# indrajeetadityaroy9/vit-bias-aware-structural-distillation

Measured on AMD Instinct MI355X. Metric: images/sec BASD train step, DeiT-T student / ViT-B teacher bs=256, higher is better.
Workload: dtype bf16; 1 GPU; BASELINE configs[1]: DeiT-Tiny/16 student, ViT-Base/16 teacher (random init), 224x224, E=4 extraction points, loss linalg fp32/fp64; global_batch=256, per_gpu_batch=256, parallelism=dp1, grad_checkpointing=False

## Files before the change

### vit-bias-aware-structural-distillation_amd/csrc/token_gram.hip

```cpp
#include "basd_frag.h"

namespace basd {

constexpr int TM = 64;
constexpr int KC = 32;
constexpr int XS = KC + 2;
constexpr int MAXCT = 8;

__device__ __forceinline__ int nct_tiles(int d_out) { const int n = d_out >> 4; return n * (n + 1) / 2; }

template <typename T>
__device__ __forceinline__ float ld_as_f32(const T* p);
template <> __device__ __forceinline__ float ld_as_f32<float>(const float* p) { return *p; }
template <> __device__ __forceinline__ float ld_as_f32<unsigned short>(const unsigned short* p) {
  return bf16_bits_to_f32(*p);
}

template <typename T, int MAXGT>
__global__ __launch_bounds__(512) void token_gram_kernel(const T* __restrict__ x, int64_t rows, int d_in,
                                                         int rows_per_batch, int64_t batch_stride,
                                                         const float* __restrict__ proj, int d_out,
                                                         double* __restrict__ gram,
                                                         double* __restrict__ colsum) {
  extern __shared__ __align__(16) float sm[];
  const int ldz = d_out + 16;
  float* Xs = sm;
  float* Ps = Xs + TM * XS;
  float* Z = Ps + d_out * XS;
  __shared__ unsigned char s_it[136], s_jt[136];
  const int tid = threadIdx.x, lane = tid & 63, wave = tid >> 6;
  const int nct = d_out >> 4;
  const int rt = wave & 3;
  const int ct0 = (wave >> 2) * ((nct + 1) >> 1);
  const int ct1 = (wave >> 2) ? nct : ((nct + 1) >> 1);
  const int ngt = nct * (nct + 1) / 2;

  for (int g = threadIdx.x; g < nct_tiles(d_out); g += 512) {
    int it = 0;
    while ((it + 1) * (it + 2) / 2 <= g) ++it;
    s_it[g] = (unsigned char)it;
    s_jt[g] = (unsigned char)(g - it * (it + 1) / 2);
  }
  __syncthreads();
  f64x4 gacc[MAXGT];
#pragma unroll
  for (int i = 0; i < MAXGT; ++i) gacc[i] = (f64x4){0.0, 0.0, 0.0, 0.0};
  double csum = 0.0;

  const int64_t ntiles = (rows + TM - 1) / TM;
  for (int64_t tile = blockIdx.x; tile < ntiles; tile += gridDim.x) {
    const int64_t r0 = tile * TM;
    f32x4 zacc[MAXCT];
#pragma unroll
    for (int i = 0; i < MAXCT; ++i) zacc[i] = (f32x4){0.f, 0.f, 0.f, 0.f};
    for (int k0 = 0; k0 < d_in; k0 += KC) {
      __syncthreads();
      for (int i = tid; i < TM * KC; i += 512) {
        const int r = i / KC, k = i - r * KC;
        const int64_t gr = r0 + r;
        const int64_t gb = gr / rows_per_batch;
        Xs[r * XS + k] = (gr < rows) ? ld_as_f32<T>(x + gb * batch_stride + (gr - gb * rows_per_batch) * d_in + k0 + k) : 0.f;
      }
      for (int i = tid; i < d_out * KC; i += 512) {
        const int r = i / KC, k = i - r * KC;
        Ps[r * XS + k] = proj[(size_t)r * d_in + k0 + k];
      }
      __syncthreads();
#pragma unroll 2
      for (int kk = 0; kk < KC / 4; ++kk) {
        const float a = Xs[(rt * 16 + (lane & 15)) * XS + kk * 4 + (lane >> 4)];
#pragma unroll
        for (int c = 0; c < MAXCT; ++c) {
          const int ct = ct0 + c;
          if (ct < ct1) {
            const float b = Ps[(ct * 16 + (lane & 15)) * XS + kk * 4 + (lane >> 4)];
            zacc[c] = __builtin_amdgcn_mfma_f32_16x16x4f32(a, b, zacc[c], 0, 0, 0);
          }
        }
      }
    }
#pragma unroll
    for (int c = 0; c < MAXCT; ++c) {
      const int ct = ct0 + c;
      if (ct < ct1) {
#pragma unroll
        for (int reg = 0; reg < 4; ++reg)
          Z[(rt * 16 + (lane >> 4) * 4 + reg) * ldz + ct * 16 + (lane & 15)] = zacc[c][reg];
      }
    }
    __syncthreads();
    if (tid < d_out) {
      double s = 0.0;
      for (int r = 0; r < TM; ++r) s += (double)Z[r * ldz + tid];
      csum += s;
    }
#pragma unroll
    for (int gi = 0; gi < MAXGT; ++gi) {
      const int g = wave + gi * 8;
      if (g < ngt) {
        const int it = s_it[g], jt = s_jt[g];
#pragma unroll 2
        for (int kk = 0; kk < TM / 4; ++kk) {
          const float* zr = Z + (kk * 4 + (lane >> 4)) * ldz + (lane & 15);
          const double a = (double)zr[it * 16];
          const double b = (double)zr[jt * 16];
          gacc[gi] = __builtin_amdgcn_mfma_f64_16x16x4f64(a, b, gacc[gi], 0, 0, 0);
        }
      }
    }
  }
#pragma unroll
  for (int gi = 0; gi < MAXGT; ++gi) {
    const int g = wave + gi * 8;
    if (g < ngt) {
      const int it = s_it[g], jt = s_jt[g];
#pragma unroll
      for (int reg = 0; reg < 4; ++reg) {
        const int i = it * 16 + (lane >> 4) + 4 * reg;
        const int j = jt * 16 + (lane & 15);
        const double v = gacc[gi][reg];
        atomicAdd(&gram[(size_t)i * d_out + j], v);
      }
    }
  }
  if (tid < d_out) atomicAdd(&colsum[tid], csum);
}

}

extern "C" int basd_token_gram(const void* x, int x_dtype, int64_t rows, int d_in, int rows_per_batch,
                               int64_t batch_stride, const float* proj, int d_out, double* gram, double* colsum,
                               void* stream) {
  using namespace basd;
  if (rows <= 0) return BASD_OK;
  if (rows_per_batch < 1) return fail(BASD_ERR_SHAPE, "token_gram: rows_per_batch < 1");
  if (d_out < 16 || d_out > 256 || d_out % 16 || d_in < KC || d_in % KC)
    return fail(BASD_ERR_SHAPE, "token_gram: need d_out %% 16 == 0, 16 <= d_out <= 256, d_in %% %d == 0 (got %d, %d)",
                KC, d_out, d_in);
  const size_t lds = (size_t)(TM * XS + d_out * XS + TM * (d_out + 16)) * 4;
  const int64_t ntiles = (rows + TM - 1) / TM;
  const int grid = (int)(ntiles < 256 ? ntiles : 256);
  hipStream_t st = (hipStream_t)stream;
#define BASD_TG_LAUNCH(T, G)                                                                        \
  do {                                                                                              \
    allow_full_lds((const void*)token_gram_kernel<T, G>);                                           \
    hipLaunchKernelGGL((token_gram_kernel<T, G>), dim3(grid), dim3(512), lds, st, (const T*)x, rows, d_in, \
                       rows_per_batch, batch_stride, proj, d_out, gram, colsum);                                                  \
  } while (0)
  if (x_dtype == BASD_DTYPE_F32) {
    if (d_out <= 192) BASD_TG_LAUNCH(float, 10); else BASD_TG_LAUNCH(float, 17);
  } else if (x_dtype == BASD_DTYPE_BF16) {
    if (d_out <= 192) BASD_TG_LAUNCH(unsigned short, 10); else BASD_TG_LAUNCH(unsigned short, 17);
  } else {
    return fail(BASD_ERR_DTYPE, "token_gram: dtype %d", x_dtype);
  }
#undef BASD_TG_LAUNCH
  return check_launch("token_gram");
}

namespace basd {

constexpr int TM2 = 128;
constexpr int KC2 = 32;
constexpr int PROW = 80;

template <int NCT>
__global__ __launch_bounds__(256) void token_gram_bf16x3_kernel(const unsigned short* __restrict__ x, int64_t rows,
                                                                int d_in, int rows_per_batch, int64_t batch_stride,
                                                                const unsigned short* __restrict__ psplit,
                                                                double* __restrict__ gram,
                                                                double* __restrict__ colsum) {
  constexpr int D_OUT = NCT * 16;
  constexpr int LDZ = D_OUT + 16;
  constexpr int NGT = NCT * (NCT + 1) / 2;
  constexpr int GT_PER_WAVE = (NGT + 3) / 4;
  extern __shared__ __align__(16) unsigned char smem[];
  unsigned char* Pl = smem;
  float* Z = reinterpret_cast<float*>(smem);
  __shared__ unsigned char s_it[NGT], s_jt[NGT];
  const int tid = threadIdx.x, lane = tid & 63, wave = tid >> 6;
  for (int g = tid; g < NGT; g += 256) {
    int it = 0;
    while ((it + 1) * (it + 2) / 2 <= g) ++it;
    s_it[g] = (unsigned char)it;
    s_jt[g] = (unsigned char)(g - it * (it + 1) / 2);
  }
  f64x4 gacc[GT_PER_WAVE];
#pragma unroll
  for (int i = 0; i < GT_PER_WAVE; ++i) gacc[i] = (f64x4){0.0, 0.0, 0.0, 0.0};
  double csum = 0.0;
  const size_t split_stride = (size_t)D_OUT * d_in;

  const int64_t ntiles = (rows + TM2 - 1) / TM2;
  for (int64_t tile = blockIdx.x; tile < ntiles; tile += gridDim.x) {
    const int64_t r0 = tile * TM2 + wave * 32;
    f32x4 zacc[2][NCT];
#pragma unroll
    for (int g = 0; g < 2; ++g)
#pragma unroll
      for (int c = 0; c < NCT; ++c) zacc[g][c] = (f32x4){0.f, 0.f, 0.f, 0.f};
    const int64_t ra = r0 + (lane & 15), rb = ra + 16;
    const int64_t ba = ra / rows_per_batch, bb = rb / rows_per_batch;
    const unsigned short* xa = x + ba * batch_stride + (ra - ba * rows_per_batch) * d_in + 8 * (lane >> 4);
    const unsigned short* xb = x + bb * batch_stride + (rb - bb * rows_per_batch) * d_in + 8 * (lane >> 4);
    constexpr int PVEC = (3 * D_OUT * 4 + 255) / 256;
    uint4 pre[PVEC];
    bf16x8 a0n, a1n;
    auto fetch = [&](int k0) {
#pragma unroll
      for (int v = 0; v < PVEC; ++v) {
        const int e = tid + 256 * v;
        const int q = e & 3, rc = e >> 2;
        const int sp = rc / D_OUT, col = rc - sp * D_OUT;
        pre[v] = (rc < 3 * D_OUT)
                     ? *reinterpret_cast<const uint4*>(psplit + sp * split_stride + (size_t)col * d_in + k0 + 8 * q)
                     : make_uint4(0, 0, 0, 0);
      }
      a0n = (bf16x8){0, 0, 0, 0, 0, 0, 0, 0};
      a1n = a0n;
      if (ra < rows) a0n = *reinterpret_cast<const bf16x8*>(xa + k0);
      if (rb < rows) a1n = *reinterpret_cast<const bf16x8*>(xb + k0);
    };
    auto stash = [&](unsigned char* buf) {
#pragma unroll
      for (int v = 0; v < PVEC; ++v) {
        const int e = tid + 256 * v;
        const int q = e & 3, rc = e >> 2;
        if (rc < 3 * D_OUT) *reinterpret_cast<uint4*>(buf + (size_t)rc * PROW + 16 * q) = pre[v];
      }
    };
    constexpr size_t PBUF = (size_t)3 * D_OUT * PROW;
    __syncthreads();
    fetch(0);
    stash(Pl);
    bf16x8 a0 = a0n, a1 = a1n;
    __syncthreads();
    int cur = 0;
    for (int k0 = 0; k0 < d_in; k0 += KC2) {
      const bool more = k0 + KC2 < d_in;
      if (more) fetch(k0 + KC2);
      const unsigned char* Pc = Pl + cur * PBUF;
#pragma unroll
      for (int s = 0; s < 3; ++s) {
#pragma unroll
        for (int c = 0; c < NCT; ++c) {
          const bf16x8 b = *reinterpret_cast<const bf16x8*>(
              Pc + (size_t)(s * D_OUT + c * 16 + (lane & 15)) * PROW + 16 * (lane >> 4));
          zacc[0][c] = __builtin_amdgcn_mfma_f32_16x16x32_bf16(a0, b, zacc[0][c], 0, 0, 0);
          zacc[1][c] = __builtin_amdgcn_mfma_f32_16x16x32_bf16(a1, b, zacc[1][c], 0, 0, 0);
        }
      }
      if (more) {
        stash(Pl + (cur ^ 1) * PBUF);
        a0 = a0n; a1 = a1n;
      }
      cur ^= 1;
      __syncthreads();
    }
    __syncthreads();
#pragma unroll
    for (int g = 0; g < 2; ++g)
#pragma unroll
      for (int c = 0; c < NCT; ++c)
#pragma unroll
        for (int reg = 0; reg < 4; ++reg)
          Z[(wave * 32 + g * 16 + (lane >> 4) * 4 + reg) * LDZ + c * 16 + (lane & 15)] = zacc[g][c][reg];
    __syncthreads();
    const int64_t rows_left = rows - tile * TM2;
    const int nvalid = rows_left < TM2 ? (int)rows_left : TM2;
    float* mu = Z + (size_t)TM2 * LDZ;
    double* wv = reinterpret_cast<double*>(mu + D_OUT);
    if (tid < D_OUT) {
      double sacc = 0.0;
      for (int r = 0; r < TM2; ++r) sacc += (double)Z[r * LDZ + tid];
      const float m_ = (float)(sacc / (double)nvalid);
      mu[tid] = m_;
      wv[tid] = sacc - 0.5 * (double)nvalid * (double)m_;
      csum += sacc;
    }
    __syncthreads();
    for (int e = tid; e < nvalid * D_OUT; e += 256) {
      const int r = e / D_OUT, c = e - r * D_OUT;
      Z[r * LDZ + c] -= mu[c];
    }
    __syncthreads();
#pragma unroll
    for (int gi = 0; gi < GT_PER_WAVE; ++gi) {
      const int g = wave + gi * 4;
      if (g < NGT) {
        const int it = s_it[g], jt = s_jt[g];
        f32x4 t = {0.f, 0.f, 0.f, 0.f};
#pragma unroll 8
        for (int kk = 0; kk < TM2 / 4; ++kk) {
          const float* zr = Z + (kk * 4 + (lane >> 4)) * LDZ + (lane & 15);
          t = __builtin_amdgcn_mfma_f32_16x16x4f32(zr[it * 16], zr[jt * 16], t, 0, 0, 0);
        }
        {
          typedef unsigned int tg_u32x2 __attribute__((ext_vector_type(2)));
          tg_u32x2 a02 = __builtin_amdgcn_permlane32_swap(__float_as_uint(t[0]), __float_as_uint(t[2]), false, false);
          tg_u32x2 a13 = __builtin_amdgcn_permlane32_swap(__float_as_uint(t[1]), __float_as_uint(t[3]), false, false);
          tg_u32x2 b01 = __builtin_amdgcn_permlane16_swap(a02[0], a13[0], false, false);
          tg_u32x2 b23 = __builtin_amdgcn_permlane16_swap(a02[1], a13[1], false, false);
          gacc[gi][0] += (double)__uint_as_float(b01[0]);
          gacc[gi][1] += (double)__uint_as_float(b01[1]);
          gacc[gi][2] += (double)__uint_as_float(b23[0]);
          gacc[gi][3] += (double)__uint_as_float(b23[1]);
        }
        const int ks = lane >> 4;
        const double mi = (double)mu[it * 16 + (lane & 15)], mj = (double)mu[jt * 16 + (lane & 15)];
        const double wi = wv[it * 16 + (lane & 15)], wj = wv[jt * 16 + (lane & 15)];
        const double ai = ks == 0 ? mi : ks == 1 ? wi : 0.0;
        const double bj = ks == 0 ? wj : ks == 1 ? mj : 0.0;
        gacc[gi] = __builtin_amdgcn_mfma_f64_16x16x4f64(ai, bj, gacc[gi], 0, 0, 0);
      }
    }
  }
#pragma unroll
  for (int gi = 0; gi < GT_PER_WAVE; ++gi) {
    const int g = wave + gi * 4;
    if (g < NGT) {
      const int it = s_it[g], jt = s_jt[g];
#pragma unroll
      for (int reg = 0; reg < 4; ++reg) {
        const int i = it * 16 + (lane >> 4) + 4 * reg;
        const int j = jt * 16 + (lane & 15);
        const double v = gacc[gi][reg];
        atomicAdd(&gram[(size_t)i * D_OUT + j], v);
      }
    }
  }
  if (tid < D_OUT) atomicAdd(&colsum[tid], csum);
}

template <int NCT>
__global__ __launch_bounds__(256) void token_gram_bf16x3_t256_kernel(const unsigned short* __restrict__ x, int64_t rows,
                                                                int d_in, int rows_per_batch, int64_t batch_stride,
                                                                const unsigned short* __restrict__ psplit,
                                                                double* __restrict__ gram,
                                                                double* __restrict__ colsum) {
  constexpr int D_OUT = NCT * 16;
  constexpr int LDZ = D_OUT + 16;
  constexpr int NGT = NCT * (NCT + 1) / 2;
  constexpr int GT_PER_WAVE = (NGT + 3) / 4;
  extern __shared__ __align__(16) unsigned char smem[];
  unsigned char* Pl = smem;
  float* Z = reinterpret_cast<float*>(smem);
  __shared__ unsigned char s_it[NGT], s_jt[NGT];
  const int tid = threadIdx.x, lane = tid & 63, wave = tid >> 6;
  for (int g = tid; g < NGT; g += 256) {
    int it = 0;
    while ((it + 1) * (it + 2) / 2 <= g) ++it;
    s_it[g] = (unsigned char)it;
    s_jt[g] = (unsigned char)(g - it * (it + 1) / 2);
  }
  double csum = 0.0;
  const size_t split_stride = (size_t)D_OUT * d_in;
  __syncthreads();

  const int64_t ntiles = (rows + 2 * TM2 - 1) / (2 * TM2);
  for (int64_t tile = blockIdx.x; tile < ntiles; tile += gridDim.x) {
    f32x4 zacc[4][NCT];
#pragma unroll
    for (int g = 0; g < 4; ++g)
#pragma unroll
      for (int c = 0; c < NCT; ++c) zacc[g][c] = (f32x4){0.f, 0.f, 0.f, 0.f};
    const unsigned short* xr[4];
    bool rok[4];
#pragma unroll
    for (int g = 0; g < 4; ++g) {
      const int64_t r = tile * (2 * TM2) + (g >> 1) * TM2 + wave * 32 + (g & 1) * 16 + (lane & 15);
      rok[g] = r < rows;
      const int64_t rr = rok[g] ? r : 0;
      const int64_t bq = rr / rows_per_batch;
      xr[g] = x + bq * batch_stride + (rr - bq * rows_per_batch) * d_in + 8 * (lane >> 4);
    }
    constexpr int PVEC = (3 * D_OUT * 4 + 255) / 256;
    uint4 pre[PVEC];
    bf16x8 an[4];
    auto fetch = [&](int k0) {
#pragma unroll
      for (int v = 0; v < PVEC; ++v) {
        const int e = tid + 256 * v;
        const int q = e & 3, rc = e >> 2;
        const int sp = rc / D_OUT, col = rc - sp * D_OUT;
        pre[v] = (rc < 3 * D_OUT)
                     ? *reinterpret_cast<const uint4*>(psplit + sp * split_stride + (size_t)col * d_in + k0 + 8 * q)
                     : make_uint4(0, 0, 0, 0);
      }
#pragma unroll
      for (int g = 0; g < 4; ++g) {
        an[g] = (bf16x8){0, 0, 0, 0, 0, 0, 0, 0};
        if (rok[g]) an[g] = *reinterpret_cast<const bf16x8*>(xr[g] + k0);
      }
    };
    auto stash = [&](unsigned char* buf) {
#pragma unroll
      for (int v = 0; v < PVEC; ++v) {
        const int e = tid + 256 * v;
        const int q = e & 3, rc = e >> 2;
        if (rc < 3 * D_OUT) *reinterpret_cast<uint4*>(buf + (size_t)rc * PROW + 16 * q) = pre[v];
      }
    };
    constexpr size_t PBUF = (size_t)3 * D_OUT * PROW;
    __syncthreads();
    fetch(0);
    stash(Pl);
    bf16x8 ac[4];
#pragma unroll
    for (int g = 0; g < 4; ++g) ac[g] = an[g];
    __syncthreads();
    int cur = 0;
    for (int k0 = 0; k0 < d_in; k0 += KC2) {
      const bool more = k0 + KC2 < d_in;
      if (more) fetch(k0 + KC2);
      const unsigned char* Pc = Pl + cur * PBUF;
#pragma unroll
      for (int s_ = 0; s_ < 3; ++s_) {
#pragma unroll
        for (int c = 0; c < NCT; ++c) {
          const bf16x8 b = *reinterpret_cast<const bf16x8*>(
              Pc + (size_t)(s_ * D_OUT + c * 16 + (lane & 15)) * PROW + 16 * (lane >> 4));
#pragma unroll
          for (int g = 0; g < 4; ++g) zacc[g][c] = __builtin_amdgcn_mfma_f32_16x16x32_bf16(ac[g], b, zacc[g][c], 0, 0, 0);
        }
      }
      if (more) {
        stash(Pl + (cur ^ 1) * PBUF);
#pragma unroll
        for (int g = 0; g < 4; ++g) ac[g] = an[g];
      }
      cur ^= 1;
      __syncthreads();
    }
    f64x4 gacc[GT_PER_WAVE];
#pragma unroll
    for (int i = 0; i < GT_PER_WAVE; ++i) gacc[i] = (f64x4){0.0, 0.0, 0.0, 0.0};
#pragma unroll
    for (int pass = 0; pass < 2; ++pass) {
    const int64_t rows_left = rows - (tile * (2 * TM2) + pass * TM2);
    if (rows_left <= 0) break;
    __syncthreads();
#pragma unroll
    for (int g = 0; g < 2; ++g)
#pragma unroll
      for (int c = 0; c < NCT; ++c)
#pragma unroll
        for (int reg = 0; reg < 4; ++reg)
          Z[(wave * 32 + g * 16 + (lane >> 4) * 4 + reg) * LDZ + c * 16 + (lane & 15)] = zacc[2 * pass + g][c][reg];
    __syncthreads();
    const int nvalid = rows_left < TM2 ? (int)rows_left : TM2;
    float* mu = Z + (size_t)TM2 * LDZ;
    double* wv = reinterpret_cast<double*>(mu + D_OUT);
    if (tid < D_OUT) {
      double sacc = 0.0;
      for (int r = 0; r < TM2; ++r) sacc += (double)Z[r * LDZ + tid];
      const float m_ = (float)(sacc / (double)nvalid);
      mu[tid] = m_;
      wv[tid] = sacc - 0.5 * (double)nvalid * (double)m_;
      csum += sacc;
    }
    __syncthreads();
    for (int e = tid; e < nvalid * D_OUT; e += 256) {
      const int r = e / D_OUT, c = e - r * D_OUT;
      Z[r * LDZ + c] -= mu[c];
    }
    __syncthreads();
#pragma unroll
    for (int gi = 0; gi < GT_PER_WAVE; ++gi) {
      const int g = wave + gi * 4;
      if (g < NGT) {
        const int it = s_it[g], jt = s_jt[g];
        f32x4 t = {0.f, 0.f, 0.f, 0.f};
#pragma unroll 8
        for (int kk = 0; kk < TM2 / 4; ++kk) {
          const float* zr = Z + (kk * 4 + (lane >> 4)) * LDZ + (lane & 15);
          t = __builtin_amdgcn_mfma_f32_16x16x4f32(zr[it * 16], zr[jt * 16], t, 0, 0, 0);
        }
        {
          typedef unsigned int tg_u32x2 __attribute__((ext_vector_type(2)));
          tg_u32x2 a02 = __builtin_amdgcn_permlane32_swap(__float_as_uint(t[0]), __float_as_uint(t[2]), false, false);
          tg_u32x2 a13 = __builtin_amdgcn_permlane32_swap(__float_as_uint(t[1]), __float_as_uint(t[3]), false, false);
          tg_u32x2 b01 = __builtin_amdgcn_permlane16_swap(a02[0], a13[0], false, false);
          tg_u32x2 b23 = __builtin_amdgcn_permlane16_swap(a02[1], a13[1], false, false);
          gacc[gi][0] += (double)__uint_as_float(b01[0]);
          gacc[gi][1] += (double)__uint_as_float(b01[1]);
          gacc[gi][2] += (double)__uint_as_float(b23[0]);
          gacc[gi][3] += (double)__uint_as_float(b23[1]);
        }
        const int ks = lane >> 4;
        const double mi = (double)mu[it * 16 + (lane & 15)], mj = (double)mu[jt * 16 + (lane & 15)];
        const double wi = wv[it * 16 + (lane & 15)], wj = wv[jt * 16 + (lane & 15)];
        const double ai = ks == 0 ? mi : ks == 1 ? wi : 0.0;
        const double bj = ks == 0 ? wj : ks == 1 ? mj : 0.0;
        gacc[gi] = __builtin_amdgcn_mfma_f64_16x16x4f64(ai, bj, gacc[gi], 0, 0, 0);
      }
    }
    }
#pragma unroll
    for (int gi = 0; gi < GT_PER_WAVE; ++gi) {
      const int g = wave + gi * 4;
      if (g < NGT) {
        const int it = s_it[g], jt = s_jt[g];
#pragma unroll
        for (int reg = 0; reg < 4; ++reg) {
          const int i = it * 16 + (lane >> 4) + 4 * reg;
          const int j = jt * 16 + (lane & 15);
          atomicAdd(&gram[(size_t)i * D_OUT + j], gacc[gi][reg]);
        }
      }
    }
  }
  if (tid < D_OUT) atomicAdd(&colsum[tid], csum);
}

template <int NCT>
static void launch_tg_bf16x3(const void* x, int64_t rows, int d_in, int rows_per_batch, int64_t batch_stride,
                             const void* psplit, double* gram, double* colsum, hipStream_t st) {
  constexpr int D_OUT = NCT * 16;
  const size_t p_bytes = (size_t)2 * 3 * D_OUT * PROW;
  const size_t z_bytes = (size_t)TM2 * (D_OUT + 16) * 4 + (size_t)D_OUT * 12;
  const size_t lds = p_bytes > z_bytes ? p_bytes : z_bytes;
  const int64_t ntiles = (rows + TM2 - 1) / TM2;
  if (ntiles > 256) {
    const int64_t nt2 = (rows + 2 * TM2 - 1) / (2 * TM2);
    const int grid2 = (int)(nt2 < 256 ? nt2 : 256);
    allow_full_lds((const void*)token_gram_bf16x3_t256_kernel<NCT>);
    hipLaunchKernelGGL((token_gram_bf16x3_t256_kernel<NCT>), dim3(grid2), dim3(256), lds, st, (const unsigned short*)x, rows,
                       d_in, rows_per_batch, batch_stride, (const unsigned short*)psplit, gram, colsum);
    return;
  }
  const int grid = (int)(ntiles < 256 ? ntiles : 256);
  allow_full_lds((const void*)token_gram_bf16x3_kernel<NCT>);
  hipLaunchKernelGGL((token_gram_bf16x3_kernel<NCT>), dim3(grid), dim3(256), lds, st, (const unsigned short*)x, rows,
                     d_in, rows_per_batch, batch_stride, (const unsigned short*)psplit, gram, colsum);
}

}

extern "C" int basd_token_gram_bf16x3(const void* x, int64_t rows, int d_in, int rows_per_batch, int64_t batch_stride,
                                      const void* proj_split, int d_out, double* gram, double* colsum,
                                      void* stream) {
  using namespace basd;
  if (rows <= 0) return BASD_OK;
  if (rows_per_batch < 1) return fail(BASD_ERR_SHAPE, "token_gram_bf16x3: rows_per_batch < 1");
  if (d_in % KC2 || d_in < KC2) return fail(BASD_ERR_SHAPE, "token_gram_bf16x3: d_in %% 32 != 0 (%d)", d_in);
  if ((((uintptr_t)x) & 15) || batch_stride % 8)
    return fail(BASD_ERR_SHAPE, "token_gram_bf16x3: need a 16-byte aligned x and batch_stride %% 8 == 0 (got %lld)",
                (long long)batch_stride);
  hipStream_t st = (hipStream_t)stream;
  switch (d_out) {
    case 32: launch_tg_bf16x3<2>(x, rows, d_in, rows_per_batch, batch_stride, proj_split, gram, colsum, st); break;
    case 64: launch_tg_bf16x3<4>(x, rows, d_in, rows_per_batch, batch_stride, proj_split, gram, colsum, st); break;
    case 128: launch_tg_bf16x3<8>(x, rows, d_in, rows_per_batch, batch_stride, proj_split, gram, colsum, st); break;
    case 192: launch_tg_bf16x3<12>(x, rows, d_in, rows_per_batch, batch_stride, proj_split, gram, colsum, st); break;
    default: return fail(BASD_ERR_SHAPE, "token_gram_bf16x3: d_out %d not in {32, 64, 128, 192}", d_out);
  }
  return check_launch("token_gram_bf16x3");
}

namespace basd {

constexpr int GW_TR = 64;
constexpr int GW_BC = 128;
constexpr int GW_LD = GW_BC + 16;

__global__ __launch_bounds__(256) __attribute__((amdgpu_waves_per_eu(2, 2))) void gram_wide_f32_kernel(const float* __restrict__ z, int64_t rows, int d, int nbc,
                                                            int rsplit, double* __restrict__ gram,
                                                            double* __restrict__ colsum) {
  extern __shared__ __align__(16) float gw_lds[];
  float* Pi = gw_lds;
  float* Pj = Pi + GW_TR * GW_LD;
  float* mu = Pj + GW_TR * GW_LD;
  double* wv = reinterpret_cast<double*>(mu + 256);
  const int tid = threadIdx.x, lane = tid & 63, wave = tid >> 6;
  const int blk = blockIdx.x / rsplit, rs = blockIdx.x - blk * rsplit;
  int bi = 0;
  while ((bi + 1) * (bi + 2) / 2 <= blk) ++bi;
  const int bj = blk - bi * (bi + 1) / 2;
  const bool diag = bi == bj;
  const int ci0 = bi * GW_BC, cj0 = bj * GW_BC;
  const int64_t ntile = (rows + GW_TR - 1) / GW_TR;
  const int64_t t_lo = ntile * rs / rsplit, t_hi = ntile * (rs + 1) / rsplit;
  f64x4 acc[2][8];
#pragma unroll
  for (int a = 0; a < 2; ++a)
#pragma unroll
    for (int b = 0; b < 8; ++b) acc[a][b] = (f64x4){0.0, 0.0, 0.0, 0.0};
  double csum = 0.0;
  const int sr = tid >> 5, sq = tid & 31;
  float4 pre_i[8], pre_j[8];
  auto fetch = [&](int64_t tile) {
    const int64_t r0 = tile * GW_TR;
#pragma unroll
    for (int p = 0; p < 8; ++p) {
      const int64_t r = r0 + sr + 8 * p;
      const bool ok = r < rows;
      const float* src = z + (ok ? r : 0) * (int64_t)d;
      const bool oki = ok && ci0 + 4 * sq < d, okj = ok && cj0 + 4 * sq < d;
      pre_i[p] = oki ? *reinterpret_cast<const float4*>(src + ci0 + 4 * sq) : make_float4(0.f, 0.f, 0.f, 0.f);
      if (!diag) pre_j[p] = okj ? *reinterpret_cast<const float4*>(src + cj0 + 4 * sq) : make_float4(0.f, 0.f, 0.f, 0.f);
    }
  };
  for (int64_t tile = t_lo; tile < t_hi; ++tile) {
    fetch(tile);
    __syncthreads();
#pragma unroll
    for (int p = 0; p < 8; ++p) {
      *reinterpret_cast<float4*>(Pi + (sr + 8 * p) * GW_LD + 4 * sq) = pre_i[p];
      if (!diag) *reinterpret_cast<float4*>(Pj + (sr + 8 * p) * GW_LD + 4 * sq) = pre_j[p];
    }
    __syncthreads();
    const int64_t left = rows - tile * GW_TR;
    const int nvalid = left < GW_TR ? (int)left : GW_TR;
    {
      const float* col = (tid < 128 ? Pi : (diag ? Pi : Pj)) + (tid & 127);
      double s = 0.0;
#pragma unroll 8
      for (int r = 0; r < GW_TR; ++r) s += (double)col[r * GW_LD];
      const float m_ = (float)(s / (double)nvalid);
      mu[tid] = m_;
      wv[tid] = s - 0.5 * (double)nvalid * (double)m_;
      if (diag && tid < 128) csum += s;
    }
    __syncthreads();
    const float* Pjj = diag ? Pi : Pj;
    const int li = lane & 15, kq = lane >> 4;
    const bool partial = nvalid < GW_TR;
#pragma unroll
    for (int a = 0; a < 2; ++a) {
      const int it = 2 * wave + a;
      const float mi = mu[it * 16 + li];
      float af[GW_TR / 4];
#pragma unroll
      for (int kk = 0; kk < GW_TR / 4; ++kk) {
        const int r = kk * 4 + kq;
        const float v = Pi[r * GW_LD + it * 16 + li] - mi;
        af[kk] = (partial && r >= nvalid) ? 0.f : v;
      }
      double mi_r[4], wi_r[4];
#pragma unroll
      for (int reg = 0; reg < 4; ++reg) { mi_r[reg] = (double)mu[it * 16 + 4 * kq + reg]; wi_r[reg] = wv[it * 16 + 4 * kq + reg]; }
#pragma unroll
      for (int jp = 0; jp < 4; ++jp) {
        const int j0 = 2 * jp, j1 = 2 * jp + 1;
        if (diag && j0 > it) continue;
        const bool use1 = !(diag && j1 > it);
        const float mj0 = mu[128 + j0 * 16 + li], mj1 = mu[128 + j1 * 16 + li];
        f32x4 t0 = {0.f, 0.f, 0.f, 0.f}, t1 = {0.f, 0.f, 0.f, 0.f};
#pragma unroll
        for (int kk = 0; kk < GW_TR / 4; ++kk) {
          const int r = kk * 4 + kq;
          float b0 = Pjj[r * GW_LD + j0 * 16 + li] - mj0, b1 = Pjj[r * GW_LD + j1 * 16 + li] - mj1;
          if (partial && r >= nvalid) { b0 = 0.f; b1 = 0.f; }
          t0 = __builtin_amdgcn_mfma_f32_16x16x4f32(af[kk], b0, t0, 0, 0, 0);
          t1 = __builtin_amdgcn_mfma_f32_16x16x4f32(af[kk], b1, t1, 0, 0, 0);
        }
        const double wj0 = wv[128 + j0 * 16 + li], wj1 = wv[128 + j1 * 16 + li];
#pragma unroll
        for (int reg = 0; reg < 4; ++reg) {
          acc[a][j0][reg] += (double)t0[reg] + mi_r[reg] * wj0 + wi_r[reg] * (double)mj0;
          if (use1) acc[a][j1][reg] += (double)t1[reg] + mi_r[reg] * wj1 + wi_r[reg] * (double)mj1;
        }
      }
    }
  }
  const int li = lane & 15, kq = lane >> 4;
#pragma unroll
  for (int a = 0; a < 2; ++a) {
    const int it = 2 * wave + a;
#pragma unroll
    for (int jt = 0; jt < 8; ++jt) {
      if (diag && jt > it) continue;
#pragma unroll
      for (int reg = 0; reg < 4; ++reg) {
        const int gi = ci0 + it * 16 + 4 * kq + reg, gj = cj0 + jt * 16 + li;
        if (gi < d && gj < d) atomicAdd(&gram[(size_t)gi * d + gj], acc[a][jt][reg]);
      }
    }
  }
  if (diag && tid < 128 && ci0 + tid < d) atomicAdd(&colsum[ci0 + tid], csum);
}

}

extern "C" int basd_gram_f32_centred(const float* z, int64_t rows, int d, double* gram, double* colsum, void* stream) {
  using namespace basd;
  if (rows <= 0) return BASD_OK;
  if (d < 16 || d % 16 || d > 4096 || (((uintptr_t)z) & 15))
    return fail(BASD_ERR_SHAPE, "gram_f32_centred: need d %% 16 == 0, 16 <= d <= 4096, 16-byte aligned z (d=%d)", d);
  const int nbc = (d + GW_BC - 1) / GW_BC;
  const int nblk = nbc * (nbc + 1) / 2;
  const int64_t ntile = (rows + GW_TR - 1) / GW_TR;
  int rsplit = 512 / nblk;
  if ((int64_t)rsplit > ntile / 8) rsplit = (int)(ntile / 8);
  if (rsplit < 1) rsplit = 1;
  const size_t lds = (size_t)2 * GW_TR * GW_LD * 4 + 256 * 4 + 256 * 8;
  allow_full_lds((const void*)gram_wide_f32_kernel);
  hipLaunchKernelGGL(gram_wide_f32_kernel, dim3(nblk * rsplit), dim3(256), lds, (hipStream_t)stream, z, rows, d, nbc,
                     rsplit, gram, colsum);
  return check_launch("gram_f32_centred");
}
```

Baseline: 8247 images/sec.

## Stream projection tiles into LDS with direct global-to-LDS loads in a three-stage ring

Replaces the register-staged double buffer for the projection split in the large-row token Gram kernel with a three-stage LDS ring. The ring is filled by global_load_lds_dwordx4 DMA using an XOR-swizzled layout, and x fragments are loaded through inline asm with counted vmcnt waits. The intent is to stop projection data passing through VGPRs and ds_write, and to overlap the next chunk's loads with the MFMAs using one barrier per chunk. In exchange it relies on fragile inline asm, m0 manipulation and manual scheduling barriers, needs more LDS, and adds a cap on d_in.

```diff
diff --git a/vit-bias-aware-structural-distillation_amd/csrc/token_gram.hip b/vit-bias-aware-structural-distillation_amd/csrc/token_gram.hip
--- a/vit-bias-aware-structural-distillation_amd/csrc/token_gram.hip
+++ b/vit-bias-aware-structural-distillation_amd/csrc/token_gram.hip
@@ -1,3 +1,4 @@
+#include <type_traits>
 #include "basd_frag.h"
 
 namespace basd {
@@ -332,6 +333,15 @@
   if (tid < D_OUT) atomicAdd(&colsum[tid], csum);
 }
 
+constexpr int TG_NS = 3;
+
+__device__ __forceinline__ int tg_swz(int byte) { return byte ^ (((byte >> 9) & 1) << 5); }
+
+template <int N>
+__device__ __forceinline__ void tg_wait_pieces(u32x4 (&x)[4]) {
+  asm volatile("s_waitcnt vmcnt(%4)" : "+v"(x[0]), "+v"(x[1]), "+v"(x[2]), "+v"(x[3]) : "n"(N) : "memory");
+}
+
 template <int NCT>
 __global__ __launch_bounds__(256) void token_gram_bf16x3_t256_kernel(const unsigned short* __restrict__ x, int64_t rows,
                                                                 int d_in, int rows_per_batch, int64_t batch_stride,
@@ -342,8 +352,12 @@
   constexpr int LDZ = D_OUT + 16;
   constexpr int NGT = NCT * (NCT + 1) / 2;
   constexpr int GT_PER_WAVE = (NGT + 3) / 4;
+  constexpr int NP = 3 * NCT;
+  constexpr int NPW = (NP + 3) / 4;
+  constexpr int STAGE = NP * 1024;
+  static_assert(TG_NS == 3, "the issue order and the counted wait of the chunk loop are written for three stages");
+  static_assert(2 * NPW + 4 < 64, "vmcnt is a 6-bit counter");
   extern __shared__ __align__(16) unsigned char smem[];
-  unsigned char* Pl = smem;
   float* Z = reinterpret_cast<float*>(smem);
   __shared__ unsigned char s_it[NGT], s_jt[NGT];
   const int tid = threadIdx.x, lane = tid & 63, wave = tid >> 6;
@@ -354,7 +368,18 @@
     s_jt[g] = (unsigned char)(g - it * (it + 1) / 2);
   }
   double csum = 0.0;
-  const size_t split_stride = (size_t)D_OUT * d_in;
+  const int wave_u = __builtin_amdgcn_readfirstlane(wave);
+  const unsigned int lds_base = (unsigned int)(size_t)smem;
+  const unsigned char* pbytes = reinterpret_cast<const unsigned char*>(psplit);
+  const int q_dma = tg_swz(lane * 16);
+  int piece[NPW];
+  unsigned int poff[NPW];
+#pragma unroll
+  for (int j = 0; j < NPW; ++j) {
+    piece[j] = (wave_u + 4 * j) % NP;
+    poff[j] = (unsigned int)(((piece[j] * 16 + (q_dma >> 6)) * (size_t)d_in + ((q_dma >> 4) & 3) * 8) * 2);
+  }
+  const int frag_off = tg_swz((lane & 15) * 64 + (lane >> 4) * 16);
   __syncthreads();
 
   const int64_t ntiles = (rows + 2 * TM2 - 1) / (2 * TM2);
@@ -374,64 +399,73 @@
       const int64_t bq = rr / rows_per_batch;
       xr[g] = x + bq * batch_stride + (rr - bq * rows_per_batch) * d_in + 8 * (lane >> 4);
     }
-    constexpr int PVEC = (3 * D_OUT * 4 + 255) / 256;
-    uint4 pre[PVEC];
-    bf16x8 an[4];
-    auto fetch = [&](int k0) {
-#pragma unroll
-      for (int v = 0; v < PVEC; ++v) {
-        const int e = tid + 256 * v;
-        const int q = e & 3, rc = e >> 2;
-        const int sp = rc / D_OUT, col = rc - sp * D_OUT;
-        pre[v] = (rc < 3 * D_OUT)
-                     ? *reinterpret_cast<const uint4*>(psplit + sp * split_stride + (size_t)col * d_in + k0 + 8 * q)
-                     : make_uint4(0, 0, 0, 0);
-      }
+    u32x4 xn[4];
+    auto load_x = [&](int k0) {
+#pragma unroll
+      for (int g = 0; g < 4; ++g)
+        asm volatile("global_load_dwordx4 %0, %1, off" : "=v"(xn[g]) : "v"(xr[g] + k0) : "memory");
+    };
+    auto issue_piece = [&](int j, int stage, const unsigned char* base_u) {
+      const unsigned int dst = lds_base + stage * STAGE + piece[j] * 1024;
+      unsigned int keep;
+      asm volatile("s_mov_b32 %0, m0\n\ts_nop 3\n\ts_mov_b32 m0, %3\n\ts_nop 0\n\tglobal_load_lds_dwordx4 %1, %2\n\ts_mov_b32 m0, %0"
+                   : "=&s"(keep) : "v"(poff[j]), "s"(base_u), "s"(dst) : "memory");
+    };
+    const int nchunks = d_in / KC2;
+    asm volatile("s_waitcnt vmcnt(0)" ::: "memory");
+    __syncthreads();
+    {
+      const int c1 = nchunks > 1 ? 1 : 0;
+#pragma unroll
+      for (int j = 0; j < NPW; ++j) issue_piece(j, 0, pbytes);
+      load_x(0);
+#pragma unroll
+      for (int j = 0; j < NPW; ++j) issue_piece(j, 1, pbytes + (size_t)c1 * (KC2 * 2));
+    }
+    int st = 0;
+#pragma nounroll
+    for (int c = 0; c < nchunks; ++c) {
+      tg_wait_pieces<NPW>(xn);
+      __builtin_amdgcn_s_barrier();
+      __builtin_amdgcn_sched_barrier(0);
+      bf16x8 ac[4];
 #pragma unroll
       for (int g = 0; g < 4; ++g) {
-        an[g] = (bf16x8){0, 0, 0, 0, 0, 0, 0, 0};
-        if (rok[g]) an[g] = *reinterpret_cast<const bf16x8*>(xr[g] + k0);
-      }
-    };
-    auto stash = [&](unsigned char* buf) {
-#pragma unroll
-      for (int v = 0; v < PVEC; ++v) {
-        const int e = tid + 256 * v;
-        const int q = e & 3, rc = e >> 2;
-        if (rc < 3 * D_OUT) *reinterpret_cast<uint4*>(buf + (size_t)rc * PROW + 16 * q) = pre[v];
-      }
-    };
-    constexpr size_t PBUF = (size_t)3 * D_OUT * PROW;
-    __syncthreads();
-    fetch(0);
-    stash(Pl);
-    bf16x8 ac[4];
-#pragma unroll
-    for (int g = 0; g < 4; ++g) ac[g] = an[g];
-    __syncthreads();
-    int cur = 0;
-    for (int k0 = 0; k0 < d_in; k0 += KC2) {
-      const bool more = k0 + KC2 < d_in;
-      if (more) fetch(k0 + KC2);
-      const unsigned char* Pc = Pl + cur * PBUF;
-#pragma unroll
-      for (int s_ = 0; s_ < 3; ++s_) {
-#pragma unroll
-        for (int c = 0; c < NCT; ++c) {
-          const bf16x8 b = *reinterpret_cast<const bf16x8*>(
-              Pc + (size_t)(s_ * D_OUT + c * 16 + (lane & 15)) * PROW + 16 * (lane >> 4));
-#pragma unroll
-          for (int g = 0; g < 4; ++g) zacc[g][c] = __builtin_amdgcn_mfma_f32_16x16x32_bf16(ac[g], b, zacc[g][c], 0, 0, 0);
-        }
-      }
-      if (more) {
-        stash(Pl + (cur ^ 1) * PBUF);
-#pragma unroll
-        for (int g = 0; g < 4; ++g) ac[g] = an[g];
-      }
-      cur ^= 1;
-      __syncthreads();
-    }
+        const u32x4 v = rok[g] ? xn[g] : (u32x4){0u, 0u, 0u, 0u};
+        ac[g] = __builtin_bit_cast(bf16x8, v);
+      }
+      const int cx = c + 1 < nchunks ? c + 1 : nchunks - 1, cp = c + 2 < nchunks ? c + 2 : nchunks - 1;
+      load_x(cx * KC2);
+      const int stn = st == 0 ? TG_NS - 1 : st - 1;
+      const unsigned char* base_n = pbytes + (size_t)cp * (KC2 * 2);
+      const unsigned char* Pc = smem + st * STAGE + frag_off;
+      bf16x8 bq[2][4];
+      auto read_block = [&](bf16x8 (&q)[4], int b) {
+#pragma unroll
+        for (int i = 0; i < 4; ++i)
+          if (4 * b + i < NP) q[i] = *reinterpret_cast<const bf16x8*>(Pc + (4 * b + i) * 1024);
+      };
+      read_block(bq[0], 0);
+#pragma unroll
+      for (int b = 0; b < NPW; ++b) {
+        __builtin_amdgcn_sched_barrier(0);
+        issue_piece(b, stn, base_n);
+        if (b + 1 < NPW) read_block(bq[(b + 1) & 1], b + 1);
+        __builtin_amdgcn_sched_barrier(0);
+#pragma unroll
+        for (int i = 0; i < 4; ++i) {
+          const int t = 4 * b + i;
+          if (t < NP) {
+#pragma unroll
+            for (int g = 0; g < 4; ++g)
+              zacc[g][t % NCT] = __builtin_amdgcn_mfma_f32_16x16x32_bf16(ac[g], bq[b & 1][i], zacc[g][t % NCT], 0, 0, 0);
+          }
+        }
+      }
+      __builtin_amdgcn_sched_barrier(0);
+      st = st == TG_NS - 1 ? 0 : st + 1;
+    }
+    asm volatile("s_waitcnt vmcnt(0)" : "+v"(xn[0]), "+v"(xn[1]), "+v"(xn[2]), "+v"(xn[3]) : : "memory");
     f64x4 gacc[GT_PER_WAVE];
 #pragma unroll
     for (int i = 0; i < GT_PER_WAVE; ++i) gacc[i] = (f64x4){0.0, 0.0, 0.0, 0.0};
@@ -524,8 +558,10 @@
   if (ntiles > 256) {
     const int64_t nt2 = (rows + 2 * TM2 - 1) / (2 * TM2);
     const int grid2 = (int)(nt2 < 256 ? nt2 : 256);
+    const size_t ring_bytes = (size_t)TG_NS * 3 * NCT * 1024;
+    const size_t lds2 = ring_bytes > z_bytes ? ring_bytes : z_bytes;
     allow_full_lds((const void*)token_gram_bf16x3_t256_kernel<NCT>);
-    hipLaunchKernelGGL((token_gram_bf16x3_t256_kernel<NCT>), dim3(grid2), dim3(256), lds, st, (const unsigned short*)x, rows,
+    hipLaunchKernelGGL((token_gram_bf16x3_t256_kernel<NCT>), dim3(grid2), dim3(256), lds2, st, (const unsigned short*)x, rows,
                        d_in, rows_per_batch, batch_stride, (const unsigned short*)psplit, gram, colsum);
     return;
   }
@@ -544,6 +580,7 @@
   if (rows <= 0) return BASD_OK;
   if (rows_per_batch < 1) return fail(BASD_ERR_SHAPE, "token_gram_bf16x3: rows_per_batch < 1");
   if (d_in % KC2 || d_in < KC2) return fail(BASD_ERR_SHAPE, "token_gram_bf16x3: d_in %% 32 != 0 (%d)", d_in);
+  if (d_in > (1 << 20)) return fail(BASD_ERR_SHAPE, "token_gram_bf16x3: d_in %d > 2^20", d_in);
   if ((((uintptr_t)x) & 15) || batch_stride % 8)
     return fail(BASD_ERR_SHAPE, "token_gram_bf16x3: need a 16-byte aligned x and batch_stride %% 8 == 0 (got %lld)",
                 (long long)batch_stride);
```

Result: no change. 8304 images/sec, median of 6 (+0.7%).
